# google/nerfactor

Hardware: AMD Instinct MI355X
Metric: rays/sec (NeRF coarse+fine render, 64+128 samples/ray) (higher is better)
Workload: dtype bf16; 1 GPU; lego_3072-shaped NeRF coarse+fine MLP render, 800x800 rays/view, 64+128 samples (BASELINE.json configs[1]); rays_per_view=640000, n_samples_coarse=64, n_samples_fine=128, kernel_variant=7

## Files before the change

### nerfactor_amd/csrc/mlp_engine.hpp

```cpp
#pragma once
#include <type_traits>
#include "nfx_common.hpp"

namespace nfx {

constexpr int kFragBytes = 1024;
constexpr int kSlotFrags = 24;
constexpr int kSlotBytes = kSlotFrags * kFragBytes;
constexpr int kPieceThreads = 256;


template <int B, int E, typename F>
__device__ __forceinline__ void static_for(F&& f) {
    if constexpr (B < E) {
        f(std::integral_constant<int, B>{});
        static_for<B + 1, E>(f);
    }
}

struct WStream {
    const u32x4* gnext;
    const u32x4* gbase;
    const u32x4* gend;
    char* ring;
    int cur;
};

template <int NL, int NW>
struct Stage {
    static constexpr int G = NW / 4;
    static constexpr int N = (NL + G - 1) / G;
    u32x4 r[N];
    __device__ __forceinline__ void load(const u32x4* g, int tid) {
        const int grp = tid >> 8, t = tid & 255;
#pragma unroll
        for (int k = 0; k < N; ++k) {
            const int i = k * G + grp;
            if ((k + 1) * G <= NL || i < NL) r[k] = g[i * kPieceThreads + t];
        }
    }
    __device__ __forceinline__ void store(u32x4* dst, int tid) const {
        const int grp = tid >> 8, t = tid & 255;
#pragma unroll
        for (int k = 0; k < N; ++k) {
            const int i = k * G + grp;
            if ((k + 1) * G <= NL || i < NL) dst[i * kPieceThreads + t] = r[k];
        }
    }
};

template <int NL, int NW>
__device__ __forceinline__ void stream_prologue(WStream& ws, int tid) {
    Stage<NL, NW> st;
    st.load(ws.gnext, tid);
    st.store(reinterpret_cast<u32x4*>(ws.ring), tid);
    ws.gnext += NL * kPieceThreads;
    ws.cur = 0;
    __syncthreads();
}

template <int NL_NEXT, int NW, typename F>
__device__ __forceinline__ void with_chunk(WStream& ws, int tid, F&& compute) {
    Stage<NL_NEXT, NW> st;
    st.load(ws.gnext, tid);
    compute(ws.ring + ws.cur * kSlotBytes);
    st.store(reinterpret_cast<u32x4*>(ws.ring + (ws.cur ^ 1) * kSlotBytes), tid);
    ws.gnext += NL_NEXT * kPieceThreads;
    if (ws.gnext == ws.gend) ws.gnext = ws.gbase;
    ws.cur ^= 1;
    __syncthreads();
}

template <int NLMAX, int NW, typename F>
__device__ __forceinline__ void with_chunk_rt(WStream& ws, int tid, int n_next, F&& compute) {
    constexpr int G = NW / 4;
    constexpr int N = (NLMAX + G - 1) / G;
    u32x4 r[N];
    const int grp = tid >> 8, t = tid & 255;
#pragma unroll
    for (int k = 0; k < N; ++k) {
        const int i = k * G + grp;
        if (i < n_next) r[k] = ws.gnext[i * kPieceThreads + t];
    }
    compute(ws.ring + ws.cur * kSlotBytes);
    u32x4* dst = reinterpret_cast<u32x4*>(ws.ring + (ws.cur ^ 1) * kSlotBytes);
#pragma unroll
    for (int k = 0; k < N; ++k) {
        const int i = k * G + grp;
        if (i < n_next) dst[i * kPieceThreads + t] = r[k];
    }
    ws.gnext += n_next * kPieceThreads;
    if (ws.gnext == ws.gend) ws.gnext = ws.gbase;
    ws.cur ^= 1;
    __syncthreads();
}

template <int CT>
__device__ __forceinline__ void bias_init(const float* bias_tile, int h, f32x16 (&acc)[CT]) {
#pragma unroll
    for (int g = 0; g < 4; ++g) {
        const f32x4 v = *reinterpret_cast<const f32x4*>(bias_tile + 8 * g + 4 * h);
#pragma unroll
        for (int c = 0; c < CT; ++c) {
            acc[c][4 * g + 0] = v[0];
            acc[c][4 * g + 1] = v[1];
            acc[c][4 * g + 2] = v[2];
            acc[c][4 * g + 3] = v[3];
        }
    }
}

template <int KS, int KSA, int CT>
__device__ __forceinline__ void mma_k(const char* lane_frag0, const bf16x8 (&b)[KSA][CT],
                                      f32x16 (&acc)[CT]) {
    static_assert(KS <= KSA, "operand array too small");
#pragma unroll
    for (int s = 0; s < KS; ++s) {
        const bf16x8 a = *reinterpret_cast<const bf16x8*>(lane_frag0 + s * kFragBytes);
#pragma unroll
        for (int c = 0; c < CT; ++c)
            acc[c] = __builtin_amdgcn_mfma_f32_32x32x16_bf16(a, b[s][c], acc[c], 0, 0, 0);
    }
}

template <int KS1, int KS2, int NL_NEXT, int NW, int KS1A, int KS2A, int CT, typename Init>
__device__ __forceinline__ void tile_init(WStream& ws, int tid, Init&& init,
                                          const bf16x8 (&b1)[KS1A][CT],
                                          const bf16x8 (&b2)[KS2A][CT], f32x16 (&acc)[CT]) {
    const int lane = tid & 63;
    init(acc);
    with_chunk<NL_NEXT, NW>(ws, tid, [&](const char* chunk) {
        const char* f0 = chunk + lane * 16;
        mma_k<KS1>(f0, b1, acc);
        if constexpr (KS2 > 0) mma_k<KS2>(f0 + KS1 * kFragBytes, b2, acc);
    });
}

template <int KS1, int KS2, int NL_NEXT, int NW, int KS1A, int KS2A, int CT>
__device__ __forceinline__ void tile_raw(WStream& ws, int tid, const float* bias_tile,
                                         const bf16x8 (&b1)[KS1A][CT],
                                         const bf16x8 (&b2)[KS2A][CT], f32x16 (&acc)[CT]) {
    const int h = (tid & 63) >> 5;
    tile_init<KS1, KS2, NL_NEXT, NW>(
        ws, tid, [&](f32x16(&a)[CT]) { bias_init<CT>(bias_tile, h, a); }, b1, b2, acc);
}

template <int CT>
__device__ __forceinline__ void vec_init(const float* __restrict__ vec_tile, int h,
                                         f32x16 (&acc)[CT]) {
#pragma unroll
    for (int g = 0; g < 4; ++g) {
        const f32x4 v = *reinterpret_cast<const f32x4*>(vec_tile + 8 * g + 4 * h);
#pragma unroll
        for (int c = 0; c < CT; ++c) {
            acc[c][4 * g + 0] = v[0];
            acc[c][4 * g + 1] = v[1];
            acc[c][4 * g + 2] = v[2];
            acc[c][4 * g + 3] = v[3];
        }
    }
}

template <bool RELU, int CT>
__device__ __forceinline__ void acc_to_b(const f32x16 (&acc)[CT], bf16x8 (&lo)[CT],
                                         bf16x8 (&hi)[CT]) {
#pragma unroll
    for (int c = 0; c < CT; ++c) {
#pragma unroll
        for (int j = 0; j < 8; ++j) {
            float v0 = acc[c][j], v1 = acc[c][8 + j];
            if (RELU) {
                v0 = __builtin_amdgcn_fmed3f(v0, 0.0f, __builtin_inff());
                v1 = __builtin_amdgcn_fmed3f(v1, 0.0f, __builtin_inff());
            }
            lo[c][j] = (__bf16)v0;
            hi[c][j] = (__bf16)v1;
        }
    }
}

template <int KS1, int KS2, int NT, int NL_SELF, int NL_NEXT, bool RELU, int NW, int KS1A,
          int KS2A, int NTA, int CT>
__device__ __forceinline__ void layer(WStream& ws, int tid, const float* bias,
                                      const bf16x8 (&b1)[KS1A][CT],
                                      const bf16x8 (&b2)[KS2A][CT], bf16x8 (&bout)[NTA][CT]) {
    static_assert(2 * NT <= NTA, "output array too small");
    static_for<0, NT>([&](auto T) {
        constexpr int t = decltype(T)::value;
        f32x16 acc[CT];
        tile_raw<KS1, KS2, (t == NT - 1 ? NL_NEXT : NL_SELF), NW>(ws, tid, bias + 32 * t, b1, b2,
                                                                 acc);
        acc_to_b<RELU, CT>(acc, bout[2 * t], bout[2 * t + 1]);
    });
}

template <int KS1, int KS2, int NT, int NLMAX, bool RELU, int NW, int KS1A, int KS2A, int NTA, int CT>
__device__ __forceinline__ void layer_rt(WStream& ws, int tid, const float* bias, int nl_self, int nl_next,
                                         const bf16x8 (&b1)[KS1A][CT], const bf16x8 (&b2)[KS2A][CT],
                                         bf16x8 (&bout)[NTA][CT]) {
    static_assert(2 * NT <= NTA, "output array too small");
    const int lane = tid & 63;
    static_for<0, NT>([&](auto T) {
        constexpr int t = decltype(T)::value;
        f32x16 acc[CT];
        bias_init<CT>(bias + 32 * t, lane >> 5, acc);
        with_chunk_rt<NLMAX, NW>(ws, tid, t == NT - 1 ? nl_next : nl_self, [&](const char* chunk) {
            const char* f0 = chunk + lane * 16;
            mma_k<KS1>(f0, b1, acc);
            if constexpr (KS2 > 0) mma_k<KS2>(f0 + KS1 * kFragBytes, b2, acc);
        });
        acc_to_b<RELU, CT>(acc, bout[2 * t], bout[2 * t + 1]);
    });
}

template <int KS1, int KS2, int NT, int NL_SELF, int NL_NEXT, bool RELU, int NW, int KS1A,
          int KS2A, int NTA, int CT>
__device__ __forceinline__ void layer_pre(WStream& ws, int tid, const float* __restrict__ pre,
                                          const bf16x8 (&b1)[KS1A][CT],
                                          const bf16x8 (&b2)[KS2A][CT], bf16x8 (&bout)[NTA][CT]) {
    static_assert(2 * NT <= NTA, "output array too small");
    const int h = (tid & 63) >> 5;
    static_for<0, NT>([&](auto T) {
        constexpr int t = decltype(T)::value;
        f32x16 acc[CT];
        tile_init<KS1, KS2, (t == NT - 1 ? NL_NEXT : NL_SELF), NW>(
            ws, tid, [&](f32x16(&a)[CT]) { vec_init<CT>(pre + 32 * t, h, a); }, b1, b2, acc);
        acc_to_b<RELU, CT>(acc, bout[2 * t], bout[2 * t + 1]);
    });
}

template <int L>
struct PeSlots {
    static constexpr int kKS = (3 * L + 2 + 7) / 8;
};

template <int L, int CT>
__device__ __forceinline__ void posenc(const float (&x)[3], int h, int c,
                                       bf16x8 (&out)[PeSlots<L>::kKS][CT]) {
    constexpr int NQ = PeSlots<L>::kKS * 8;
    float v[NQ];
#pragma unroll
    for (int q = 3 * L; q < NQ; ++q) v[q] = q == 3 * L ? (h ? x[2] : x[0]) : (q == 3 * L + 1 && !h) ? x[1] : 0.0f;
    if constexpr (L <= 4) {
#pragma unroll
        for (int q = 0; q < 3 * L; ++q) v[q] = sin_shifted_small(x[q % 3] * (float)(1 << (q / 3)), h);
    } else {
#pragma unroll
        for (int d = 0; d < 3; ++d)
#pragma unroll
            for (int k0 = 0; k0 < L; k0 += 5) {
                float sn, cs;
                sincos_cw(x[d] * (float)(1 << k0), sn, cs);
#pragma unroll
                for (int k = k0; k < k0 + 5 && k < L; ++k) {
                    v[3 * k + d] = h ? cs : sn;
                    const float s2 = 2.0f * sn * cs;
                    cs = fmaf(-2.0f * sn, sn, 1.0f);
                    sn = s2;
                }
            }
    }
#pragma unroll
    for (int s = 0; s < PeSlots<L>::kKS; ++s) {
#pragma unroll
        for (int j = 0; j < 8; ++j) out[s][c][j] = (__bf16)v[8 * s + j];
    }
}

}
```

### nerfactor_amd/csrc/nerf_mlp_v6.hip

```cpp
#include "mlp_engine.hpp"
#include "lds_dma.hpp"
#include "nerf_layout.hpp"
#include "nerf_fold_layout.hpp"

#ifdef NFX_V6_SIGMA
#define NFX_V6_NS v6s
#else
#define NFX_V6_NS v6
#endif

namespace nfx {
namespace NFX_V6_NS {

constexpr int kNW = 4, kCT = 2;
template <int DMA, bool FOLD = false> constexpr int ring_of = DMA == 1 ? 6 : FOLD ? 4 : 3;
template <int DMA, bool FOLD> constexpr int slot_of(int k) {
    if (!FOLD) return k % ring_of<DMA>;
    return DMA == 1 ? (k < 66 ? k % 6 : k - 65) : (k == 69 ? 3 : k % 3);
}
constexpr int kDmaDist = 3;
template <int DMA> constexpr int dist_of = DMA == 1 ? kDmaDist : DMA ? 3 : 2;
template <int DMA, bool FOLD = false> constexpr int lds_of = ring_of<DMA, FOLD> * kSlotBytes + nerf::kBiasFloats * 4;
#ifdef NFX_V6_SIGMA
constexpr int kNChunks = 66;
#else
constexpr int kNChunks = nerf::kNChunks;
#endif
static_assert(kNChunks % 6 == 0, "the chunk sequence wraps on the 6-slot (and the 3-slot) ring");
template <bool FOLD> constexpr int n_chunks = FOLD ? nerf::fold::kNChunks : kNChunks;
template <bool FOLD> constexpr int seq_frags(int k) { return FOLD ? nerf::fold::chunk_frags(k) : nerf::chunk_frags(k); }
template <bool FOLD> constexpr int seq_frag_offset(int k) {
    return FOLD ? nerf::fold::chunk_frag_offset(k) : nerf::chunk_frag_offset(k);
}

constexpr int kPreA = 3;

struct Acc {
    f32x16 v[kCT];
};
struct Pre {
    bf16x8 a[kPreA];
};

template <bool RELU>
__device__ __forceinline__ void cvt_pair(float v0, float v1, bf16x8& dst, int j) {
    typedef short s2 __attribute__((ext_vector_type(2)));
    typedef __bf16 b2 __attribute__((ext_vector_type(2)));
    typedef float f2 __attribute__((ext_vector_type(2)));
    const f2 vv = {v0, v1};
    b2 pr = __builtin_convertvector(vv, b2);
    if (RELU) {
        s2 w = __builtin_bit_cast(s2, pr);
        const s2 z = {0, 0};
        w = __builtin_elementwise_max(w, z);
        pr = __builtin_bit_cast(b2, w);
    }
    dst[j] = pr[0];
    dst[j + 1] = pr[1];
}

template <bool RELU>
struct EpiB {
    const Acc& acc;
    bf16x8 (&lo)[kCT];
    bf16x8 (&hi)[kCT];
    template <int R0, int R1>
    __device__ __forceinline__ void run() {
#pragma unroll
        for (int r = R0; r < R1; r += 2)
#pragma unroll
            for (int c = 0; c < kCT; ++c) {
                if (r < 8) cvt_pair<RELU>(acc.v[c][r], acc.v[c][r + 1], lo[c], r);
                else cvt_pair<RELU>(acc.v[c][r], acc.v[c][r + 1], hi[c], r - 8);
            }
    }
    __device__ __forceinline__ void finish() {
    }
};
struct EpiNone {
    template <int R0, int R1>
    __device__ __forceinline__ void run() {}
    __device__ __forceinline__ void finish() {}
};
struct EpiSigma {
    const Acc& acc;
    float (&sigma)[kCT];
    template <int R0, int R1>
    __device__ __forceinline__ void run() {
        if constexpr (R0 == 0) {
#pragma unroll
            for (int c = 0; c < kCT; ++c) sigma[c] = acc.v[c][0];
        }
    }
    __device__ __forceinline__ void finish() {}
};

__device__ __forceinline__ void bias_to_acc(const float* bias_tile, int lane, Acc& acc) {
    const float* bt = bias_tile + 4 * (lane >> 5);
#pragma unroll
    for (int g = 0; g < 4; ++g) {
        const f32x4 v = *reinterpret_cast<const f32x4*>(bt + 8 * g);
#pragma unroll
        for (int c = 0; c < kCT; ++c) {
            acc.v[c][4 * g + 0] = v[0];
            acc.v[c][4 * g + 1] = v[1];
            acc.v[c][4 * g + 2] = v[2];
            acc.v[c][4 * g + 3] = v[3];
        }
    }
}

typedef __attribute__((address_space(1))) u32x4 gu32x4;

struct Regs {
    u32x4 r[2][6];
};

struct Ctx {
    char* smem;
    const char* blob;
    int tid;
    unsigned smem_lds;
    int wave;
};

constexpr int used_frags(int k, bool fold = false) {
    return k < 8 ? 4 : k < 40 ? 16 : k < 48 ? 20 : k < (fold ? 65 : 73) ? 16 : k < (fold ? 69 : 77) ? 18 : 8;
}
constexpr int dma_pieces(int k, bool fold = false) { return (used_frags(k, fold) + kNW - 1) / kNW; }
template <int K, bool FOLD>
__device__ __forceinline__ void dma_chunk(const Ctx& cx) {
    constexpr int n = dma_pieces(K, FOLD);
    unsigned long long base = reinterpret_cast<unsigned long long>(cx.blob);
    unsigned lds = cx.smem_lds;
    asm volatile("" : "+s"(base), "+s"(lds));
    const int piece0 = cx.wave * n;
    const char* g = reinterpret_cast<const char*>(base) + (size_t)seq_frag_offset<FOLD>(K) * kFragBytes + piece0 * 1024;
    const unsigned l = lds + slot_of<1, FOLD>(K) * kSlotBytes + piece0 * 1024;
    lds_dma_pieces<n>((cx.tid & 63) * 16, g, l);
}
template <int K, int KS1, int KS2, int AB, int DMA, bool FOLD = false, int KS1A, int KS2A, typename Epi>
__device__ __forceinline__ void tile(const Ctx& cx, Regs& rg, const float* next_bias, const bf16x8 (&b1)[KS1A][kCT],
                                     const bf16x8 (&b2)[KS2A][kCT], Acc& acc, Acc& acc_next, Pre& pre, Epi&& prev) {
    constexpr int KS = KS1 + KS2;
    constexpr int PIECES = KS >= 16 ? 8 : 4;
    constexpr int EOFF = 0;
    constexpr int SP = (PIECES < KS ? PIECES : KS - 1) + EOFF;
    constexpr int K1 = (K + 1) % n_chunks<FOLD>, K2 = (K + dist_of<DMA>) % n_chunks<FOLD>;
    constexpr int NL2 = seq_frags<FOLD>(K2) / 4;
    const int lane = cx.tid & 63;
    const char* f0 = cx.smem + slot_of<DMA, FOLD>(K) * kSlotBytes + lane * 16;
    Stage<DMA ? 1 : NL2, kNW> st;
    if constexpr (DMA == 1 && !(AB & 1)) {
        dma_chunk<K2, FOLD>(cx);
    } else if constexpr (DMA == 2 && !(AB & 1)) {
        unsigned long long gb = reinterpret_cast<unsigned long long>(cx.blob);
        asm volatile("" : "+s"(gb));
        const gu32x4* g = reinterpret_cast<const gu32x4*>(gb + (size_t)seq_frag_offset<FOLD>(K2) * kFragBytes);
#pragma unroll
        for (int k = 0; k < NL2; ++k) rg.r[K & 1][k] = g[k * kPieceThreads + cx.tid];
    } else if constexpr (!(AB & 1)) {
        unsigned long long gb = reinterpret_cast<unsigned long long>(cx.blob);
        asm volatile("" : "+s"(gb));
        const gu32x4* g = reinterpret_cast<const gu32x4*>(gb + (size_t)seq_frag_offset<FOLD>(K2) * kFragBytes);
#pragma unroll
        for (int k = 0; k < NL2; ++k) st.r[k] = g[k * kPieceThreads + cx.tid];
    }
    bf16x8 abuf[kPreA + 1];
#pragma unroll
    for (int i = 0; i < kPreA; ++i) abuf[i] = pre.a[i];
    static_for<0, KS>([&](auto S) {
        constexpr int s = decltype(S)::value;
        if constexpr (s + kPreA < KS && !(AB & 8))
            abuf[(s + kPreA) % (kPreA + 1)] = *reinterpret_cast<const bf16x8*>(f0 + (s + kPreA) * kFragBytes);
        const bf16x8 a = abuf[s % (kPreA + 1)];
#pragma unroll
        for (int c = 0; c < kCT; ++c) {
            const bf16x8 b = s < KS1 ? b1[s < KS1 ? s : 0][c] : b2[s >= KS1 ? s - KS1 : 0][c];
            if constexpr (AB & 4) {
                asm volatile("" ::"v"(a), "v"(b));
            } else {
                acc.v[c] = __builtin_amdgcn_mfma_f32_32x32x16_bf16(a, b, acc.v[c], 0, 0, 0);
            }
        }
        if constexpr (EOFF > 0 && s == EOFF)
            __builtin_amdgcn_sched_barrier(0x4 | 0x10 | 0x80);
        if constexpr (s >= EOFF && s - EOFF < PIECES)
            prev.template run<16 * (s - EOFF) / PIECES, 16 * (s - EOFF + 1) / PIECES>();
        if constexpr (s == SP) {
            if constexpr (!(AB & 64)) bias_to_acc(next_bias, lane, acc_next);
            prev.finish();
        }
    });
    if constexpr (DMA == 1 && !(AB & 1)) {
        constexpr int kInFlight = dma_pieces(K2, FOLD) + (kDmaDist == 4 ? dma_pieces((K + 3) % n_chunks<FOLD>, FOLD) : 0);
        asm volatile("s_waitcnt vmcnt(%0)" ::"n"(kInFlight) : "memory");
    } else if constexpr (DMA == 2 && !(AB & 1)) {
        constexpr int KP = (K + 2) % n_chunks<FOLD>, NLP = seq_frags<FOLD>(KP) / 4;
        u32x4* dst = reinterpret_cast<u32x4*>(cx.smem + slot_of<DMA, FOLD>(KP) * kSlotBytes);
#pragma unroll
        for (int k = 0; k < NLP; ++k) dst[k * kPieceThreads + cx.tid] = rg.r[(K + 1) & 1][k];
    } else if constexpr (!(AB & 1)) {
        st.store(reinterpret_cast<u32x4*>(cx.smem + slot_of<DMA, FOLD>(K2) * kSlotBytes), cx.tid);
    }
    if constexpr (!(AB & 8)) {
        const char* f1 = cx.smem + slot_of<DMA, FOLD>(K1) * kSlotBytes + lane * 16;
#pragma unroll
        for (int i = 0; i < kPreA; ++i) pre.a[i] = *reinterpret_cast<const bf16x8*>(f1 + i * kFragBytes);
    }
    if constexpr (!(AB & 2)) asm volatile("s_barrier" ::: "memory");
}

template <int K0, int KS1, int KS2, int NT, bool RELU, int AB, int DMA, bool FOLD = false, int KS1A, int KS2A, int NTA, typename Epi0>
__device__ __forceinline__ void layer(const Ctx& cx, Regs& rg, const float* bias, const float* next_bias,
                                      const bf16x8 (&b1)[KS1A][kCT], const bf16x8 (&b2)[KS2A][kCT],
                                      bf16x8 (&bout)[NTA][kCT], Acc (&accs)[2], Pre& pre, Epi0&& prev0) {
    static_for<0, NT>([&](auto T) {
        constexpr int t = decltype(T)::value;
        constexpr int K = K0 + t;
        const float* nb = t == NT - 1 ? next_bias : bias + 32 * (t + 1);
        if constexpr (t == 0) {
            tile<K, KS1, KS2, AB, DMA, FOLD>(cx, rg, nb, b1, b2, accs[K & 1], accs[(K + 1) & 1], pre, prev0);
        } else {
                EpiB<RELU> e{accs[(K - 1) & 1], bout[2 * (t - 1)], bout[2 * (t - 1) + 1]};
                tile<K, KS1, KS2, AB, DMA, FOLD>(cx, rg, nb, b1, b2, accs[K & 1], accs[(K + 1) & 1], pre, e);
        }
    });
}

#ifndef NFX_V6_SIGMA
template <int AB, int DMA, bool FOLD>
__device__ __forceinline__ void nerf_mlp_bf16_v6_body(
    const float* __restrict__ rayo, const float* __restrict__ rayd, const float* __restrict__ zbuf, long long n_pts,
    int n_samples, const char* __restrict__ blob, float4* __restrict__ out) {
    extern __shared__ __attribute__((aligned(16))) char smem[];
    using namespace nerf;
    const int tid = threadIdx.x, lane = tid & 63, wave = tid >> 6, h = lane >> 5, p = lane & 31;
    constexpr int kTilePts = kNW * 32 * kCT;
    float* bias_lds = reinterpret_cast<float*>(smem + ring_of<DMA, FOLD> * kSlotBytes);
    {
        const float* bsrc = reinterpret_cast<const float*>(blob + (FOLD ? nerf::fold::kWeightBytes : nerf::kWeightBytes));
        for (int i = tid; i < kBiasFloats; i += kNW * 64) bias_lds[i] = bsrc[i];
    }
    typedef __attribute__((address_space(3))) char lds_char;
    Ctx cx{smem, blob, tid, (unsigned)__builtin_amdgcn_readfirstlane((unsigned)(uintptr_t)(lds_char*)smem),
           __builtin_amdgcn_readfirstlane(tid >> 6)};
    Acc accs[2];
    Pre pre;
    Regs rg;
    if constexpr (DMA == 2) {
        const u32x4* g = reinterpret_cast<const u32x4*>(blob + (size_t)seq_frag_offset<FOLD>(2) * kFragBytes);
#pragma unroll
        for (int k = 0; k < seq_frags<FOLD>(2) / 4; ++k) rg.r[1][k] = g[k * kPieceThreads + tid];
    }
    {
        Stage<seq_frags<FOLD>(0) / 4, kNW> s0;
        Stage<seq_frags<FOLD>(1) / 4, kNW> s1;
        s0.load(reinterpret_cast<const u32x4*>(blob), tid);
        s1.load(reinterpret_cast<const u32x4*>(blob + (size_t)seq_frag_offset<FOLD>(1) * kFragBytes), tid);
        s0.store(reinterpret_cast<u32x4*>(smem), tid);
        s1.store(reinterpret_cast<u32x4*>(smem + kSlotBytes), tid);
        if constexpr (DMA == 1) {
            Stage<seq_frags<FOLD>(2) / 4, kNW> s2;
            s2.load(reinterpret_cast<const u32x4*>(blob + (size_t)seq_frag_offset<FOLD>(2) * kFragBytes), tid);
            s2.store(reinterpret_cast<u32x4*>(smem + 2 * kSlotBytes), tid);
            if constexpr (kDmaDist == 4) {
                Stage<seq_frags<FOLD>(3) / 4, kNW> s3;
                s3.load(reinterpret_cast<const u32x4*>(blob + (size_t)seq_frag_offset<FOLD>(3) * kFragBytes), tid);
                s3.store(reinterpret_cast<u32x4*>(smem + 3 * kSlotBytes), tid);
            }
        }
        __syncthreads();
#pragma unroll
        for (int i = 0; i < kPreA; ++i) pre.a[i] = *reinterpret_cast<const bf16x8*>(smem + lane * 16 + i * kFragBytes);
        bias_to_acc(bias_lds + kBiasL0, lane, accs[0]);
    }
    const long long n_tiles = (n_pts + kTilePts - 1) / kTilePts;
    for (long long tl = blockIdx.x; tl < n_tiles; tl += gridDim.x) {
        bf16x8 pe[4][kCT], pv[2][kCT];
        long long m[kCT];
#pragma unroll
        for (int c = 0; c < kCT; ++c) {
            m[c] = tl * kTilePts + wave * (32 * kCT) + c * 32 + p;
            const long long mm = m[c] < n_pts ? m[c] : n_pts - 1;
            const long long ray = mm / n_samples;
            const float zz = zbuf[mm];
            float x[3], d[3];
#pragma unroll
            for (int k = 0; k < 3; ++k) {
                d[k] = rayd[ray * 3 + k];
                x[k] = rayo[ray * 3 + k] + d[k] * zz;
            }
            posenc<10, kCT>(x, h, c, pe);
            posenc<4, kCT>(d, h, c, pv);
        }
        bf16x8 ha[16][kCT], hb[16][kCT], r0[8][kCT];
        float sigma[kCT];
        const float* bl = bias_lds + kBiasL0;
        auto pend = [&](auto relu_tag, const Acc& a, bf16x8(&lo)[kCT], bf16x8(&hi)[kCT]) {
            return EpiB<decltype(relu_tag)::value>{a, lo, hi};
        };
        using T = std::true_type;
        using F = std::false_type;
        layer<0, 4, 0, 8, true, AB, DMA, FOLD>(cx, rg, bl, bl + 256 * 1, pe, pe, ha, accs, pre, EpiNone{});
        layer<8, 16, 0, 8, true, AB, DMA, FOLD>(cx, rg, bl + 256 * 1, bl + 256 * 2, ha, pe, hb, accs, pre, pend(T{}, accs[1], ha[14], ha[15]));
        layer<16, 16, 0, 8, true, AB, DMA, FOLD>(cx, rg, bl + 256 * 2, bl + 256 * 3, hb, pe, ha, accs, pre, pend(T{}, accs[1], hb[14], hb[15]));
        layer<24, 16, 0, 8, true, AB, DMA, FOLD>(cx, rg, bl + 256 * 3, bl + 256 * 4, ha, pe, hb, accs, pre, pend(T{}, accs[1], ha[14], ha[15]));
        layer<32, 16, 0, 8, true, AB, DMA, FOLD>(cx, rg, bl + 256 * 4, bl + 256 * 5, hb, pe, ha, accs, pre, pend(T{}, accs[1], hb[14], hb[15]));
        layer<40, 16, 4, 8, true, AB, DMA, FOLD>(cx, rg, bl + 256 * 5, bl + 256 * 6, ha, pe, hb, accs, pre, pend(T{}, accs[1], ha[14], ha[15]));
        layer<48, 16, 0, 8, true, AB, DMA, FOLD>(cx, rg, bl + 256 * 6, bl + 256 * 7, hb, pe, ha, accs, pre, pend(T{}, accs[1], hb[14], hb[15]));
        if constexpr (FOLD) {
        layer<56, 16, 0, 8, true, AB, DMA, FOLD>(cx, rg, bl + 256 * 7, bias_lds + kBiasBott + 256, ha, pe, hb, accs, pre, pend(T{}, accs[1], ha[14], ha[15]));
        tile<64, 16, 0, AB, DMA, FOLD>(cx, rg, bias_lds + kBiasRgb0, hb, pe, accs[0], accs[1], pre, pend(T{}, accs[1], hb[14], hb[15]));
        {
            EpiSigma es{accs[0], sigma};
            layer<65, 16, 2, 4, true, AB, DMA, FOLD>(cx, rg, bias_lds + kBiasRgb0, bias_lds + kBiasRgb1, hb, pv, r0, accs, pre, es);
        }
        tile<69, 8, 0, AB, DMA, FOLD>(cx, rg, bl, r0, pe, accs[1], accs[0], pre, pend(T{}, accs[0], r0[6], r0[7]));
        } else {
        layer<56, 16, 0, 8, true, AB, DMA, FOLD>(cx, rg, bl + 256 * 7, bias_lds + kBiasBott, ha, pe, hb, accs, pre, pend(T{}, accs[1], ha[14], ha[15]));
        layer<64, 16, 0, 8, false, AB, DMA, FOLD>(cx, rg, bias_lds + kBiasBott, bias_lds + kBiasBott + 256, hb, pe, ha, accs, pre,
                                       pend(T{}, accs[1], hb[14], hb[15]));
        tile<72, 16, 0, AB, DMA, FOLD>(cx, rg, bias_lds + kBiasRgb0, hb, pe, accs[0], accs[1], pre, pend(F{}, accs[1], ha[14], ha[15]));
        {
            EpiSigma es{accs[0], sigma};
            layer<73, 16, 2, 4, true, AB, DMA, FOLD>(cx, rg, bias_lds + kBiasRgb0, bias_lds + kBiasRgb1, ha, pv, r0, accs, pre, es);
        }
        tile<77, 8, 0, AB, DMA, FOLD>(cx, rg, bl, r0, pe, accs[1], accs[0], pre, pend(T{}, accs[0], r0[6], r0[7]));
        }
        if (h == 0) {
#pragma unroll
            for (int c = 0; c < kCT; ++c)
                if (m[c] < n_pts) out[m[c]] = make_float4(accs[1].v[c][0], accs[1].v[c][1], accs[1].v[c][2], sigma[c]);
        }
    }
}


template <int AB, int DMA>
__global__ __launch_bounds__(kNW * 64, 1) void nerf_mlp_bf16_v6_kernel(
    const float* __restrict__ rayo, const float* __restrict__ rayd, const float* __restrict__ zbuf, long long n_pts,
    int n_samples, const char* __restrict__ blob, float4* __restrict__ out) {
    nerf_mlp_bf16_v6_body<AB, DMA, false>(rayo, rayd, zbuf, n_pts, n_samples, blob, out);
}

namespace fold {
template <int AB, int DMA>
__global__ __launch_bounds__(kNW * 64, 1) void nerf_mlp_bf16_v6_kernel(
    const float* __restrict__ rayo, const float* __restrict__ rayd, const float* __restrict__ zbuf, long long n_pts,
    int n_samples, const char* __restrict__ blob, float4* __restrict__ out) {
    nerf_mlp_bf16_v6_body<AB, DMA, true>(rayo, rayd, zbuf, n_pts, n_samples, blob, out);
}
}

#endif
}
}

#ifndef NFX_V6_SIGMA
template <int AB, int DMA, bool FOLD = false>
static int launch_v6(const float* rayo, const float* rayd, const float* z, long long n_pts, int n_samples,
                     const void* blob, float* out, int max_blocks, hipStream_t stream) {
    using namespace nfx;
    const int tile_pts = v6::kNW * 32 * v6::kCT;
    const long long n_tiles = (n_pts + tile_pts - 1) / tile_pts;
    const int grid = (int)(n_tiles < max_blocks ? n_tiles : max_blocks);
    auto kern = FOLD ? v6::fold::nerf_mlp_bf16_v6_kernel<AB, DMA> : v6::nerf_mlp_bf16_v6_kernel<AB, DMA>;
    constexpr int lds = v6::lds_of<DMA, FOLD>;
    hipError_t e = hipFuncSetAttribute(reinterpret_cast<const void*>(kern), hipFuncAttributeMaxDynamicSharedMemorySize, lds);
    if (e != hipSuccess) return (int)e;
    hipLaunchKernelGGL(kern, dim3(grid), dim3(v6::kNW * 64), lds, stream, rayo, rayd, z, n_pts, n_samples,
                       (const char*)blob, (float4*)out);
    return (int)hipGetLastError();
}

extern "C" int nfx_launch_nerf_mlp_bf16_v6(const float* rayo, const float* rayd, const float* z, long long n_pts,
                                           int n_samples, const void* blob, float* out, int max_blocks, int dma_mode,
                                           hipStream_t stream) {
    if (n_pts <= 0) return 0;
    if (dma_mode == 1) return launch_v6<0, 1>(rayo, rayd, z, n_pts, n_samples, blob, out, max_blocks, stream);
    if (dma_mode == 2) return launch_v6<0, 2>(rayo, rayd, z, n_pts, n_samples, blob, out, max_blocks, stream);
    return launch_v6<0, 0>(rayo, rayd, z, n_pts, n_samples, blob, out, max_blocks, stream);
}

extern "C" int nfx_launch_nerf_mlp_bf16_v6_fold(const float* rayo, const float* rayd, const float* z, long long n_pts,
                                                int n_samples, const void* blob, float* out, int max_blocks, int dma_mode,
                                                hipStream_t stream) {
    if (n_pts <= 0) return 0;
    if (dma_mode == 1) return launch_v6<0, 1, true>(rayo, rayd, z, n_pts, n_samples, blob, out, max_blocks, stream);
    if (dma_mode == 2) return launch_v6<0, 2, true>(rayo, rayd, z, n_pts, n_samples, blob, out, max_blocks, stream);
    return launch_v6<0, 0, true>(rayo, rayd, z, n_pts, n_samples, blob, out, max_blocks, stream);
}
#endif
```

Before: 5.248 million rays/s.

## Prefetch next tile's ray inputs and spread positional encoding across MFMA tiles

The per-tile prologue (index division, global loads of z/ray origin/direction, 10-frequency positional encoding) is moved into the previous tile's MLP pass. Index math runs in tile 48, loads are issued in tile 49 and consumed in tile 50, and the encoding is split into small pieces scheduled into spare MFMA slots of layers 6-7. View-direction encoding is deferred to the view layer. Integer division by n_samples is replaced with a double-precision reciprocal plus correction. This hides load latency and ALU work under matrix ops, at the cost of higher register pressure and more complex scheduling.

```diff
diff --git a/nerfactor_amd/csrc/mlp_engine.hpp b/nerfactor_amd/csrc/mlp_engine.hpp
--- a/nerfactor_amd/csrc/mlp_engine.hpp
+++ b/nerfactor_amd/csrc/mlp_engine.hpp
@@ -267,4 +267,51 @@
     }
 }
 
-}
+__device__ __forceinline__ long long point_div(long long m, int s) {
+    long long q = (long long)((double)m / (double)s);
+    const long long r = m - q * s;
+    q += r >= s ? 1 : 0;
+    q -= r < 0 ? 1 : 0;
+    return q;
+}
+
+template <int CT>
+struct Posenc10Pieces {
+    static constexpr int kPieces = 17;
+    float x[3], sn[3], cs[3], even;
+
+    template <int Q>
+    __device__ __forceinline__ void slot(float v, int c, bf16x8 (&out)[4][CT]) {
+        if constexpr (Q % 2 == 0) {
+            even = v;
+        } else {
+            out[Q / 8][c][Q % 8 - 1] = (__bf16)even;
+            out[Q / 8][c][Q % 8] = (__bf16)v;
+        }
+    }
+    template <int P>
+    __device__ __forceinline__ void piece(int h, int c, bf16x8 (&out)[4][CT]) {
+        static_assert(P >= 0 && P < kPieces, "piece index");
+        if constexpr (P < 3) {
+            sincos_cw(x[P] * (float)(1 << 0), sn[P], cs[P]);
+        } else if constexpr (P >= 8 && P < 11) {
+            sincos_cw(x[P - 8] * (float)(1 << 5), sn[P - 8], cs[P - 8]);
+        } else if constexpr (P < 16) {
+            constexpr int k = P < 8 ? P - 3 : P - 6;
+            static_for<0, 3>([&](auto D) {
+                constexpr int d = decltype(D)::value;
+                slot<3 * k + d>(h ? cs[d] : sn[d], c, out);
+                if constexpr (k % 5 != 4) {
+                    const float s2 = 2.0f * sn[d] * cs[d];
+                    cs[d] = fmaf(-2.0f * sn[d], sn[d], 1.0f);
+                    sn[d] = s2;
+                }
+            });
+        } else {
+            slot<30>(h ? x[2] : x[0], c, out);
+            slot<31>(h ? 0.0f : x[1], c, out);
+        }
+    }
+};
+
+}
diff --git a/nerfactor_amd/csrc/nerf_mlp_v6.hip b/nerfactor_amd/csrc/nerf_mlp_v6.hip
--- a/nerfactor_amd/csrc/nerf_mlp_v6.hip
+++ b/nerfactor_amd/csrc/nerf_mlp_v6.hip
@@ -82,6 +82,14 @@
     __device__ __forceinline__ void run() {}
     __device__ __forceinline__ void finish() {}
 };
+struct FillNone {
+    template <int K>
+    __device__ __forceinline__ void issue() {}
+    template <int K, int S>
+    __device__ __forceinline__ void run() {}
+    template <int K>
+    __device__ __forceinline__ void landed() {}
+};
 struct EpiSigma {
     const Acc& acc;
     float (&sigma)[kCT];
@@ -139,9 +147,9 @@
     const unsigned l = lds + slot_of<1, FOLD>(K) * kSlotBytes + piece0 * 1024;
     lds_dma_pieces<n>((cx.tid & 63) * 16, g, l);
 }
-template <int K, int KS1, int KS2, int AB, int DMA, bool FOLD = false, int KS1A, int KS2A, typename Epi>
+template <int K, int KS1, int KS2, int AB, int DMA, bool FOLD = false, int KS1A, int KS2A, typename Epi, typename Fill>
 __device__ __forceinline__ void tile(const Ctx& cx, Regs& rg, const float* next_bias, const bf16x8 (&b1)[KS1A][kCT],
-                                     const bf16x8 (&b2)[KS2A][kCT], Acc& acc, Acc& acc_next, Pre& pre, Epi&& prev) {
+                                     const bf16x8 (&b2)[KS2A][kCT], Acc& acc, Acc& acc_next, Pre& pre, Epi&& prev, Fill& fill) {
     constexpr int KS = KS1 + KS2;
     constexpr int PIECES = KS >= 16 ? 8 : 4;
     constexpr int EOFF = 0;
@@ -166,6 +174,7 @@
 #pragma unroll
         for (int k = 0; k < NL2; ++k) st.r[k] = g[k * kPieceThreads + cx.tid];
     }
+    fill.template issue<K>();
     bf16x8 abuf[kPreA + 1];
 #pragma unroll
     for (int i = 0; i < kPreA; ++i) abuf[i] = pre.a[i];
@@ -191,6 +200,7 @@
             if constexpr (!(AB & 64)) bias_to_acc(next_bias, lane, acc_next);
             prev.finish();
         }
+        fill.template run<K, s>();
     });
     if constexpr (DMA == 1 && !(AB & 1)) {
         constexpr int kInFlight = dma_pieces(K2, FOLD) + (kDmaDist == 4 ? dma_pieces((K + 3) % n_chunks<FOLD>, FOLD) : 0);
@@ -203,6 +213,7 @@
     } else if constexpr (!(AB & 1)) {
         st.store(reinterpret_cast<u32x4*>(cx.smem + slot_of<DMA, FOLD>(K2) * kSlotBytes), cx.tid);
     }
+    fill.template landed<K>();
     if constexpr (!(AB & 8)) {
         const char* f1 = cx.smem + slot_of<DMA, FOLD>(K1) * kSlotBytes + lane * 16;
 #pragma unroll
@@ -210,23 +221,121 @@
     }
     if constexpr (!(AB & 2)) asm volatile("s_barrier" ::: "memory");
 }
-
-template <int K0, int KS1, int KS2, int NT, bool RELU, int AB, int DMA, bool FOLD = false, int KS1A, int KS2A, int NTA, typename Epi0>
+template <int K, int KS1, int KS2, int AB, int DMA, bool FOLD = false, int KS1A, int KS2A, typename Epi>
+__device__ __forceinline__ void tile(const Ctx& cx, Regs& rg, const float* next_bias, const bf16x8 (&b1)[KS1A][kCT],
+                                     const bf16x8 (&b2)[KS2A][kCT], Acc& acc, Acc& acc_next, Pre& pre, Epi&& prev) {
+    FillNone none;
+    tile<K, KS1, KS2, AB, DMA, FOLD>(cx, rg, next_bias, b1, b2, acc, acc_next, pre, prev, none);
+}
+
+template <int K0, int KS1, int KS2, int NT, bool RELU, int AB, int DMA, bool FOLD = false, int KS1A, int KS2A, int NTA, typename Epi0,
+          typename Fill>
 __device__ __forceinline__ void layer(const Ctx& cx, Regs& rg, const float* bias, const float* next_bias,
                                       const bf16x8 (&b1)[KS1A][kCT], const bf16x8 (&b2)[KS2A][kCT],
-                                      bf16x8 (&bout)[NTA][kCT], Acc (&accs)[2], Pre& pre, Epi0&& prev0) {
+                                      bf16x8 (&bout)[NTA][kCT], Acc (&accs)[2], Pre& pre, Epi0&& prev0, Fill& fill) {
     static_for<0, NT>([&](auto T) {
         constexpr int t = decltype(T)::value;
         constexpr int K = K0 + t;
         const float* nb = t == NT - 1 ? next_bias : bias + 32 * (t + 1);
         if constexpr (t == 0) {
-            tile<K, KS1, KS2, AB, DMA, FOLD>(cx, rg, nb, b1, b2, accs[K & 1], accs[(K + 1) & 1], pre, prev0);
+            tile<K, KS1, KS2, AB, DMA, FOLD>(cx, rg, nb, b1, b2, accs[K & 1], accs[(K + 1) & 1], pre, prev0, fill);
         } else {
                 EpiB<RELU> e{accs[(K - 1) & 1], bout[2 * (t - 1)], bout[2 * (t - 1) + 1]};
-                tile<K, KS1, KS2, AB, DMA, FOLD>(cx, rg, nb, b1, b2, accs[K & 1], accs[(K + 1) & 1], pre, e);
+                tile<K, KS1, KS2, AB, DMA, FOLD>(cx, rg, nb, b1, b2, accs[K & 1], accs[(K + 1) & 1], pre, e, fill);
         }
     });
 }
+template <int K0, int KS1, int KS2, int NT, bool RELU, int AB, int DMA, bool FOLD = false, int KS1A, int KS2A, int NTA, typename Epi0>
+__device__ __forceinline__ void layer(const Ctx& cx, Regs& rg, const float* bias, const float* next_bias,
+                                      const bf16x8 (&b1)[KS1A][kCT], const bf16x8 (&b2)[KS2A][kCT],
+                                      bf16x8 (&bout)[NTA][kCT], Acc (&accs)[2], Pre& pre, Epi0&& prev0) {
+    FillNone none;
+    layer<K0, KS1, KS2, NT, RELU, AB, DMA, FOLD>(cx, rg, bias, next_bias, b1, b2, bout, accs, pre, prev0, none);
+}
+
+#ifndef NFX_V6_SIGMA
+template <bool FOLD, bool ENC>
+struct FillNext {
+    const float* __restrict__ rayo;
+    const float* __restrict__ rayd;
+    const float* __restrict__ zbuf;
+    long long n_pts;
+    int n_samples;
+    long long m_next;
+    int h;
+    const float (&d)[kCT][3];
+    float (&dn)[kCT][3];
+    bf16x8 (&pe)[4][kCT];
+    bf16x8 (&pv)[2][kCT];
+    long long mm[kCT], ray3[kCT];
+    float zz[kCT], ro[kCT][3];
+    Posenc10Pieces<kCT> enc[kCT];
+
+    static constexpr int kIndexTile = 48, kLoadTile = 49, kLandTile = 50, kEncTile = 51, kViewTile = FOLD ? 64 : 72;
+    static constexpr int slots_of(int piece) { return piece < 3 || (piece >= 8 && piece < 11) ? 3 : 1; }
+    static constexpr int kSlot0 = 8, kSlotsPerTile = 16 - kSlot0;
+    static constexpr int work_at(int slot) {
+        int at = 0;
+        for (int c = 0; c < kCT; ++c)
+            for (int piece = 0; piece < Posenc10Pieces<kCT>::kPieces; ++piece) {
+                if (at == slot) return piece * kCT + c;
+                at += slots_of(piece);
+            }
+        return -1;
+    }
+    static constexpr int kEncSlots = kCT * (6 * slots_of(0) + 11 * slots_of(3));
+    static_assert(work_at(kEncSlots - slots_of(16)) >= 0 && work_at(kEncSlots) == -1, "kEncSlots is the last slot's end");
+    static_assert(kEncTile + (kEncSlots - 1) / kSlotsPerTile < 64, "the encoding ends inside layers 6 and 7");
+
+    template <int K>
+    __device__ __forceinline__ void issue() {
+        if constexpr (K == kLoadTile) {
+#pragma unroll
+            for (int c = 0; c < kCT; ++c) {
+                zz[c] = zbuf[mm[c]];
+#pragma unroll
+                for (int k = 0; k < 3; ++k) {
+                    dn[c][k] = rayd[ray3[c] + k];
+                    ro[c][k] = rayo[ray3[c] + k];
+                }
+            }
+        }
+    }
+    template <int K, int S>
+    __device__ __forceinline__ void run() {
+        if constexpr (K == kIndexTile && (S == 8 || S == 12)) {
+            constexpr int c = (S - 8) / 4;
+            long long m = m_next + c * 32;
+            asm volatile("" : "+v"(m));
+            mm[c] = m < n_pts ? m : n_pts - 1;
+            ray3[c] = point_div(mm[c], n_samples) * 3;
+        }
+        if constexpr (K == kViewTile && (S == 8 || S == 12)) posenc<4, kCT>(d[(S - 8) / 4], h, (S - 8) / 4, pv);
+        if constexpr (ENC && K >= kEncTile && K < 64 && S >= kSlot0) {
+            constexpr int w = work_at((K - kEncTile) * kSlotsPerTile + S - kSlot0);
+            if constexpr (w >= 0) enc[w % kCT].template piece<w / kCT>(h, w % kCT, pe);
+        }
+    }
+    template <int K>
+    __device__ __forceinline__ void landed() {
+        if constexpr (ENC && K == kEncTile + (kEncSlots - 1) / kSlotsPerTile) {
+#pragma unroll
+            for (int s = 0; s < 4; ++s)
+#pragma unroll
+                for (int c = 0; c < kCT; ++c) asm volatile("" : "+v"(pe[s][c]));
+        }
+        if constexpr (K == kLandTile) {
+#pragma unroll
+            for (int c = 0; c < kCT; ++c) {
+                asm volatile("" : "+v"(zz[c]), "+v"(dn[c][0]), "+v"(dn[c][1]), "+v"(dn[c][2]), "+v"(ro[c][0]), "+v"(ro[c][1]),
+                             "+v"(ro[c][2]));
+#pragma unroll
+                for (int k = 0; k < 3; ++k) enc[c].x[k] = ro[c][k] + dn[c][k] * zz[c];
+            }
+        }
+    }
+};
+#endif
 
 #ifndef NFX_V6_SIGMA
 template <int AB, int DMA, bool FOLD>
@@ -276,24 +385,29 @@
         bias_to_acc(bias_lds + kBiasL0, lane, accs[0]);
     }
     const long long n_tiles = (n_pts + kTilePts - 1) / kTilePts;
+    constexpr bool kEncUnder = DMA == 1 || (DMA == 0 && FOLD);
+    bf16x8 pe[4][kCT];
+    float d[kCT][3], dn[kCT][3];
+#pragma unroll
+    for (int c = 0; c < kCT; ++c) {
+        const long long m0 = (long long)blockIdx.x * kTilePts + wave * (32 * kCT) + c * 32 + p;
+        const long long mm = m0 < n_pts ? m0 : n_pts - 1;
+        const long long ray = point_div(mm, n_samples);
+        const float zz = zbuf[mm];
+        float x[3];
+#pragma unroll
+        for (int k = 0; k < 3; ++k) {
+            d[c][k] = rayd[ray * 3 + k];
+            x[k] = rayo[ray * 3 + k] + d[c][k] * zz;
+        }
+        posenc<10, kCT>(x, h, c, pe);
+    }
     for (long long tl = blockIdx.x; tl < n_tiles; tl += gridDim.x) {
-        bf16x8 pe[4][kCT], pv[2][kCT];
+        bf16x8 pv[2][kCT];
         long long m[kCT];
 #pragma unroll
-        for (int c = 0; c < kCT; ++c) {
-            m[c] = tl * kTilePts + wave * (32 * kCT) + c * 32 + p;
-            const long long mm = m[c] < n_pts ? m[c] : n_pts - 1;
-            const long long ray = mm / n_samples;
-            const float zz = zbuf[mm];
-            float x[3], d[3];
-#pragma unroll
-            for (int k = 0; k < 3; ++k) {
-                d[k] = rayd[ray * 3 + k];
-                x[k] = rayo[ray * 3 + k] + d[k] * zz;
-            }
-            posenc<10, kCT>(x, h, c, pe);
-            posenc<4, kCT>(d, h, c, pv);
-        }
+        for (int c = 0; c < kCT; ++c) m[c] = tl * kTilePts + wave * (32 * kCT) + c * 32 + p;
+        FillNext<FOLD, kEncUnder> fill{rayo, rayd, zbuf, n_pts, n_samples, m[0] + (long long)gridDim.x * kTilePts, h, d, dn, pe, pv};
         bf16x8 ha[16][kCT], hb[16][kCT], r0[8][kCT];
         float sigma[kCT];
         const float* bl = bias_lds + kBiasL0;
@@ -302,36 +416,44 @@
         };
         using T = std::true_type;
         using F = std::false_type;
-        layer<0, 4, 0, 8, true, AB, DMA, FOLD>(cx, rg, bl, bl + 256 * 1, pe, pe, ha, accs, pre, EpiNone{});
-        layer<8, 16, 0, 8, true, AB, DMA, FOLD>(cx, rg, bl + 256 * 1, bl + 256 * 2, ha, pe, hb, accs, pre, pend(T{}, accs[1], ha[14], ha[15]));
-        layer<16, 16, 0, 8, true, AB, DMA, FOLD>(cx, rg, bl + 256 * 2, bl + 256 * 3, hb, pe, ha, accs, pre, pend(T{}, accs[1], hb[14], hb[15]));
-        layer<24, 16, 0, 8, true, AB, DMA, FOLD>(cx, rg, bl + 256 * 3, bl + 256 * 4, ha, pe, hb, accs, pre, pend(T{}, accs[1], ha[14], ha[15]));
-        layer<32, 16, 0, 8, true, AB, DMA, FOLD>(cx, rg, bl + 256 * 4, bl + 256 * 5, hb, pe, ha, accs, pre, pend(T{}, accs[1], hb[14], hb[15]));
-        layer<40, 16, 4, 8, true, AB, DMA, FOLD>(cx, rg, bl + 256 * 5, bl + 256 * 6, ha, pe, hb, accs, pre, pend(T{}, accs[1], ha[14], ha[15]));
-        layer<48, 16, 0, 8, true, AB, DMA, FOLD>(cx, rg, bl + 256 * 6, bl + 256 * 7, hb, pe, ha, accs, pre, pend(T{}, accs[1], hb[14], hb[15]));
+        layer<0, 4, 0, 8, true, AB, DMA, FOLD>(cx, rg, bl, bl + 256 * 1, pe, pe, ha, accs, pre, EpiNone{}, fill);
+        layer<8, 16, 0, 8, true, AB, DMA, FOLD>(cx, rg, bl + 256 * 1, bl + 256 * 2, ha, pe, hb, accs, pre, pend(T{}, accs[1], ha[14], ha[15]), fill);
+        layer<16, 16, 0, 8, true, AB, DMA, FOLD>(cx, rg, bl + 256 * 2, bl + 256 * 3, hb, pe, ha, accs, pre, pend(T{}, accs[1], hb[14], hb[15]), fill);
+        layer<24, 16, 0, 8, true, AB, DMA, FOLD>(cx, rg, bl + 256 * 3, bl + 256 * 4, ha, pe, hb, accs, pre, pend(T{}, accs[1], ha[14], ha[15]), fill);
+        layer<32, 16, 0, 8, true, AB, DMA, FOLD>(cx, rg, bl + 256 * 4, bl + 256 * 5, hb, pe, ha, accs, pre, pend(T{}, accs[1], hb[14], hb[15]), fill);
+        layer<40, 16, 4, 8, true, AB, DMA, FOLD>(cx, rg, bl + 256 * 5, bl + 256 * 6, ha, pe, hb, accs, pre, pend(T{}, accs[1], ha[14], ha[15]), fill);
+        layer<48, 16, 0, 8, true, AB, DMA, FOLD>(cx, rg, bl + 256 * 6, bl + 256 * 7, hb, pe, ha, accs, pre, pend(T{}, accs[1], hb[14], hb[15]), fill);
         if constexpr (FOLD) {
-        layer<56, 16, 0, 8, true, AB, DMA, FOLD>(cx, rg, bl + 256 * 7, bias_lds + kBiasBott + 256, ha, pe, hb, accs, pre, pend(T{}, accs[1], ha[14], ha[15]));
-        tile<64, 16, 0, AB, DMA, FOLD>(cx, rg, bias_lds + kBiasRgb0, hb, pe, accs[0], accs[1], pre, pend(T{}, accs[1], hb[14], hb[15]));
+        layer<56, 16, 0, 8, true, AB, DMA, FOLD>(cx, rg, bl + 256 * 7, bias_lds + kBiasBott + 256, ha, pe, hb, accs, pre, pend(T{}, accs[1], ha[14], ha[15]), fill);
+        tile<64, 16, 0, AB, DMA, FOLD>(cx, rg, bias_lds + kBiasRgb0, hb, pe, accs[0], accs[1], pre, pend(T{}, accs[1], hb[14], hb[15]), fill);
         {
             EpiSigma es{accs[0], sigma};
-            layer<65, 16, 2, 4, true, AB, DMA, FOLD>(cx, rg, bias_lds + kBiasRgb0, bias_lds + kBiasRgb1, hb, pv, r0, accs, pre, es);
-        }
-        tile<69, 8, 0, AB, DMA, FOLD>(cx, rg, bl, r0, pe, accs[1], accs[0], pre, pend(T{}, accs[0], r0[6], r0[7]));
+            layer<65, 16, 2, 4, true, AB, DMA, FOLD>(cx, rg, bias_lds + kBiasRgb0, bias_lds + kBiasRgb1, hb, pv, r0, accs, pre, es, fill);
+        }
+        tile<69, 8, 0, AB, DMA, FOLD>(cx, rg, bl, r0, pe, accs[1], accs[0], pre, pend(T{}, accs[0], r0[6], r0[7]), fill);
         } else {
-        layer<56, 16, 0, 8, true, AB, DMA, FOLD>(cx, rg, bl + 256 * 7, bias_lds + kBiasBott, ha, pe, hb, accs, pre, pend(T{}, accs[1], ha[14], ha[15]));
+        layer<56, 16, 0, 8, true, AB, DMA, FOLD>(cx, rg, bl + 256 * 7, bias_lds + kBiasBott, ha, pe, hb, accs, pre, pend(T{}, accs[1], ha[14], ha[15]), fill);
         layer<64, 16, 0, 8, false, AB, DMA, FOLD>(cx, rg, bias_lds + kBiasBott, bias_lds + kBiasBott + 256, hb, pe, ha, accs, pre,
-                                       pend(T{}, accs[1], hb[14], hb[15]));
-        tile<72, 16, 0, AB, DMA, FOLD>(cx, rg, bias_lds + kBiasRgb0, hb, pe, accs[0], accs[1], pre, pend(F{}, accs[1], ha[14], ha[15]));
+                                       pend(T{}, accs[1], hb[14], hb[15]), fill);
+        tile<72, 16, 0, AB, DMA, FOLD>(cx, rg, bias_lds + kBiasRgb0, hb, pe, accs[0], accs[1], pre, pend(F{}, accs[1], ha[14], ha[15]), fill);
         {
             EpiSigma es{accs[0], sigma};
-            layer<73, 16, 2, 4, true, AB, DMA, FOLD>(cx, rg, bias_lds + kBiasRgb0, bias_lds + kBiasRgb1, ha, pv, r0, accs, pre, es);
-        }
-        tile<77, 8, 0, AB, DMA, FOLD>(cx, rg, bl, r0, pe, accs[1], accs[0], pre, pend(T{}, accs[0], r0[6], r0[7]));
+            layer<73, 16, 2, 4, true, AB, DMA, FOLD>(cx, rg, bias_lds + kBiasRgb0, bias_lds + kBiasRgb1, ha, pv, r0, accs, pre, es, fill);
+        }
+        tile<77, 8, 0, AB, DMA, FOLD>(cx, rg, bl, r0, pe, accs[1], accs[0], pre, pend(T{}, accs[0], r0[6], r0[7]), fill);
         }
         if (h == 0) {
 #pragma unroll
             for (int c = 0; c < kCT; ++c)
                 if (m[c] < n_pts) out[m[c]] = make_float4(accs[1].v[c][0], accs[1].v[c][1], accs[1].v[c][2], sigma[c]);
+        }
+#pragma unroll
+        for (int c = 0; c < kCT; ++c)
+#pragma unroll
+            for (int k = 0; k < 3; ++k) d[c][k] = dn[c][k];
+        if constexpr (!kEncUnder) {
+#pragma unroll
+            for (int c = 0; c < kCT; ++c) posenc<10, kCT>(fill.enc[c].x, h, c, pe);
         }
     }
 }
```

Measured after the change: 5.290 million rays/s, median of 6. Within noise of the previous version (+0.8%).
